# BUTSpeechFIT/DiariZen

Hardware: AMD Instinct MI355X
Metric: audio-seconds/s (RTF) for wavlm-large-s80 pipeline, 16 kHz mono (higher is better)
Workload: dtype f32 (operands split into 2 fp16 terms with exact power-of-two scaling = 22 significant bits, 3 fp16 MFMA products, fp32 accumulate: the error-corrected '3xFP16/3xTF32' scheme; kernels without an fp16 variant use the 3-term bf16 split)

## Files before the change

### diarizen_amd/_lib.py

```python
from __future__ import annotations

import ctypes as C
import os
from pathlib import Path

DZN_MAX_CONV = 8
DZN_MAX_LAYERS = 32
DZN_MAX_HEADS = 16

DZN_PREC_F32 = 0
DZN_PREC_BF16 = 1
DZN_PREC_F32_SPLIT = 2
DZN_PREC_F32_H2 = 3
DZN_PREC_F16 = 4

DZN_ACT_NONE, DZN_ACT_GELU, DZN_ACT_SWISH, DZN_ACT_RELU = 0, 1, 2, 3

DZN_F32, DZN_F64, DZN_I64 = 0, 1, 2

ERRORS = {0: "ok", -1: "invalid argument", -2: "out of memory", -3: "HIP runtime error",
          -4: "bad call order", -5: "missing state_dict key"}


class DznError(RuntimeError):
# ... 127 lines not shown
            f"{p} not found: build the HIP extension first (python -m diarizen_amd.build). "
            "diarizen_amd has no CPU fallback.")
    try:
        import torch
    except Exception:
        pass
    lib = C.CDLL(str(p))
    vp, i32, i64, f32 = C.c_void_p, C.c_int32, C.c_int64, C.c_float

    def sig(name, res, args):
        fn = getattr(lib, name)
        fn.restype = res
        fn.argtypes = args

    sig("dzn_create", i32, [C.POINTER(DznConfig), C.POINTER(vp)])
    sig("dzn_load_tensor", i32, [vp, C.c_char_p, vp, C.POINTER(i64), i32, i32])
    sig("dzn_finalize_weights", i32, [vp])
    sig("dzn_num_frames", i32, [vp, i32])
    sig("dzn_segment_forward", i32, [vp, vp, i32, i32, vp, vp, vp])
    sig("dzn_segment_forward_soft", i32, [vp, vp, i32, i32, vp, vp, vp, vp])
    sig("dzn_embed_forward", i32, [vp, vp, vp, i32, i32, i32, i32, vp, vp])
    sig("dzn_embed_forward_strided", i32, [vp, vp, i64, vp, i32, i32, i32, i32, vp, vp])
    sig("dzn_prepare_masks", i32, [vp, vp, i32, i32, i32, i32, i32, vp, vp, vp])
    sig("dzn_speaker_count", i32, [vp, i32, i32, i32, vp, i32, vp, vp, vp])
    sig("dzn_cluster_activations", i32, [vp, vp, i32, i32, i32, vp, i32, i32, vp, vp])
    sig("dzn_detect", i32, [vp, i32, i32, i32, vp, vp, i32, i32, f32, f32, vp, vp, vp])
    sig("dzn_detect_range", i32, [vp, i32, i32, i32, vp, vp, i32, i32, i32, f32, f32, vp, vp, vp, vp])
    sig("dzn_diarize_range", i32, [vp, vp, i32, i32, i32, vp, i32, i32, i32, i32, vp, vp, vp, vp])
    sig("dzn_diarize_range_scores", i32, [vp, vp, vp, i32, i32, i32, vp, vp, vp, i32, i32, i32, i32, vp, vp, vp, vp, vp])
    sig("dzn_speaker_scores", i32, [vp, vp, i32, i32, i32, vp, vp, vp, i32, i32, vp, vp])
    sig("dzn_match_counts", i32, [vp, vp, i32, i32, i32, i32, i32, vp, i32, i32, vp, vp])
    sig("dzn_debug_fetch", i32, [vp, C.c_char_p, vp, i64, C.POINTER(i64)])
    sig("dzn_embed_skip_stats", i32, [vp, C.POINTER(i64), C.POINTER(i64)])
    sig("dzn_num_ignored", i32, [vp])
    sig("dzn_workspace_bytes", i64, [vp])
    sig("dzn_last_error", C.c_char_p, [vp])
    sig("dzn_destroy", i32, [vp])
    sig("dzn_version", C.c_char_p, [])
    sig("dzn_profile_enable", i32, [i32])
    sig("dzn_profile_collect", i32, [C.POINTER(DznProfEntry), i32, C.POINTER(i32)])
    sig("dzn_profile_reserve", i32, [i32])
    sig("dzn_op_relpos_bucket", i32, [i32, i32, i32])
    sig("dzn_linkage_centroid", i32, [vp, i32, i32, vp, i32])
    sig("dzn_cdist_cosine", i32, [vp, i32, i32, vp, i32, vp, i32])
    sig("dzn_link_speakers", i32, [vp, vp, i32, i32, C.c_double, vp, C.POINTER(i32), i32])
    sig("dzn_link_speakers_last", i32, [C.POINTER(i64), C.POINTER(i32), C.POINTER(i32), C.POINTER(f32)])
# ... 74 lines not shown
    sig("dzn_op_ws_accum", i32, [vp, vp, f32, i32, i64, vp])
    sig("dzn_op_ws_sum", i32, [C.POINTER(vp), C.POINTER(f32), i32, vp, i64, vp])
    sig("dzn_op_col_scale", i32, [vp, i64, i32, i64, vp, vp])
    sig("dzn_op_layernorm_t", i32, [vp, i64, vp, i64, vp, vp, vp, i64, i32, i32, f32, i32, vp, i64, vp])
    sig("dzn_op_wave_stats", i32, [vp, i32, i32, f32, vp, vp])
    sig("dzn_op_frame_prep", i32, [vp, i32, i64, i32, i32, i32, i32, vp, f32, vp, vp])
    sig("dzn_op_power", i32, [vp, i64, i32, vp, vp])
    sig("dzn_op_log_cmn", i32, [vp, i32, i32, i32, f32, vp])
    sig("dzn_op_log_cmn_gather", i32, [vp, i32, vp, i32, i32, i32, f32, vp])
    sig("dzn_op_stem_conv", i32, [vp, i32, i32, i32, i32, vp, vp, vp, vp, vp, vp, vp])
    sig("dzn_op_stats_pool", i32, [vp, i32, i32, i32, i32, vp, i32, i32, vp, vp, vp])
    sig("dzn_op_window_active", i32, [vp, i32, i32, vp, vp])
    sig("dzn_op_compact_active", i32, [vp, i32, vp, vp, vp, vp])
    if hasattr(lib, "dzn_op_posconv_resident"):
        sig("dzn_op_pad_rows_split2", i32, [vp, vp, i64, i32, i32, i32, i32, i32, vp, vp, i32, i32, vp])
        sig("dzn_op_posconv_resident", i32, [C.POINTER(DznGemmDesc), i32, i32, i32, vp])
        sig("dzn_op_posconv_resident_fits", i32, [i32, i32, i32])
    _LIB = lib
    return lib


EXPORTED = [
    "dzn_create", "dzn_load_tensor", "dzn_finalize_weights", "dzn_num_frames",
    "dzn_segment_forward", "dzn_segment_forward_soft", "dzn_embed_forward", "dzn_embed_forward_strided", "dzn_prepare_masks", "dzn_speaker_count", "dzn_cluster_activations", "dzn_detect", "dzn_detect_range", "dzn_diarize_range", "dzn_diarize_range_scores", "dzn_speaker_scores", "dzn_match_counts", "dzn_debug_fetch", "dzn_embed_skip_stats", "dzn_num_ignored",
    "dzn_workspace_bytes", "dzn_last_error", "dzn_destroy", "dzn_version", "dzn_linkage_centroid", "dzn_cdist_cosine", "dzn_host_workspace_release",
    "dzn_host_workspace_bytes", "dzn_link_speakers", "dzn_link_speakers_last",
    "dzn_flac_info", "dzn_flac_decode", "dzn_resample", "dzn_resample_tile", "dzn_decode", "dzn_beamform_delays", "dzn_beamform_sum", "dzn_beamform_tile", "dzn_decode_planar", "dzn_beamform_track", "dzn_beamform_feed", "dzn_ingest_many", "dzn_beamform_many", "dzn_gather_windows", "dzn_vbx_create", "dzn_vbx_stats", "dzn_vbx_estep", "dzn_vbx_gamma", "dzn_vbx_destroy",
    "dzn_gallery_create", "dzn_gallery_put", "dzn_gallery_drop", "dzn_gallery_search", "dzn_gallery_geometry", "dzn_gallery_rows",
    "dzn_gallery_last_launch_ms", "dzn_gallery_destroy",
    "dzn_registry_create", "dzn_registry_append", "dzn_registry_match", "dzn_registry_rows", "dzn_registry_last_launch_ms",
    "dzn_registry_destroy",
    "dzn_op_gemm", "dzn_op_split_weights", "dzn_op_split_weights_h2", "dzn_op_split_weights_mx", "dzn_op_set_gemm_mx_cfg", "dzn_checked_status", "dzn_op_set_gemm_cfg", "dzn_op_amax", "dzn_op_conv3x3_c32", "dzn_op_conv3x3_c32_h2", "dzn_op_resblock32_fused", "dzn_op_resblock_ws", "dzn_op_set_resblock_np", "dzn_op_conv3x3_c32_ex", "dzn_op_resblock32_fused_ex", "dzn_op_resblock_ws_ex", "dzn_op_set_attention_noskip", "dzn_op_split_rows", "dzn_op_layernorm", "dzn_op_row_stats", "dzn_op_gate", "dzn_op_gate_stats", "dzn_op_gate_heads", "dzn_op_stats_finalize", "dzn_op_attention", "dzn_op_attention_h2", "dzn_op_attention_planes", "dzn_op_set_attention_qb", "dzn_op_set_attention_prefetch",
    "dzn_profile_enable", "dzn_profile_collect", "dzn_profile_reserve", "dzn_op_relpos_bucket",
    "dzn_op_glu_dwconv", "dzn_op_classify", "dzn_op_groupnorm_gelu", "dzn_op_gn_stats_floats", "dzn_op_pad_rows", "dzn_op_ws_accum",
    "dzn_op_ws_sum", "dzn_op_col_scale", "dzn_op_layernorm_t", "dzn_op_wave_stats", "dzn_op_frame_prep", "dzn_op_power",
    "dzn_op_log_cmn", "dzn_op_log_cmn_gather", "dzn_op_stem_conv", "dzn_op_stats_pool", "dzn_op_window_active",
    "dzn_op_compact_active", "dzn_op_pad_rows_split2", "dzn_op_posconv_resident", "dzn_op_posconv_resident_fits",
    "dzn_op_conv0_lnq", "dzn_op_conv0", "dzn_op_split_weights_h2_frag", "dzn_op_conv01_fused",
]


def profile_enable(on: bool) -> None:
    check(load().dzn_profile_enable(int(on)), None, "dzn_profile_enable")


def profile_reserve(n_events: int) -> None:
    check(load().dzn_profile_reserve(int(n_events)), None, "dzn_profile_reserve")
# ... 25 lines not shown
```

### diarizen_amd/csrc/common.h

```cpp
#pragma once
#include <hip/hip_runtime.h>
#include <stdint.h>
#include <math.h>
#include <string.h>
#include "../../include/dzn.h"
#include "../../include/dzn_ops.h"

typedef float f32x4 __attribute__((ext_vector_type(4)));
typedef __bf16 bf16x8 __attribute__((ext_vector_type(8)));
typedef __bf16 bf16x4 __attribute__((ext_vector_type(4)));
typedef unsigned short u16;

#define DZN_WAVE 64

template <int CTRL, int ROW_MASK>
__device__ __forceinline__ float dpp_add(float v) {
  const int t = __builtin_amdgcn_update_dpp(ROW_MASK == 0xF ? __float_as_int(v) : 0, __float_as_int(v), CTRL,
                                            ROW_MASK, 0xF, false);
  return v + __int_as_float(t);
}
__device__ __forceinline__ float wave_sum(float v) {
  v = dpp_add<0xB1, 0xF>(v);
  v = dpp_add<0x4E, 0xF>(v);
  v = dpp_add<0x124, 0xF>(v);
// ... 160 lines not shown

int launch_resblock32_fused(const float* in, float* out, const void* W1, const float* cs1, const float* b1, const void* W2,
                            const float* cs2, const float* b2, const float* amax_in, float* amax_out, float l1max1,
                            float bmax1, int B, int Hs, int Ws, int np, hipStream_t s, const int* z_count = nullptr,
                            const int* z_list = nullptr);

int launch_resblock_ws(const float* in, float* out, const void* W1, const float* cs1, const float* b1, const void* W2,
                       const float* cs2, const float* b2, const float* amax_in, float* amax_out, float l1max1, float bmax1,
                       int B, int Hs, int Ws, int C, hipStream_t s, const int* z_count = nullptr, const int* z_list = nullptr,
                       int np = 2);

int op_resblock_np();

int launch_prepare_masks(const uint8_t* ml, int B, int L, int S, int median, int exclude_overlap,
                         int min_num_frames, uint8_t* filtered, float* masks, hipStream_t st);

size_t resample_lds_bytes(int o, int n, int width);
int launch_resample(const void* src, int format, int channels, int channel, int64_t src_first, int64_t src_len, int64_t T,
                    const float* bank, int o, int n, int width, int64_t m0, int64_t m1, float* dst, hipStream_t st);
int launch_decode(const void* src, int format, int channels, int channel, int64_t frames, float* dst, hipStream_t st);
int launch_ingest_many(const void* stage, const dzn_ingest_desc* desc, int num_desc, int64_t tiles, size_t lds_bytes,
                       double bytes_moved, const float* banks, float* pool, hipStream_t st);
int launch_gather_windows(const float* pool, const int64_t* offsets, int B, int window, float* dst, hipStream_t st);
int launch_beamform_delays(const float* x, int channels, int64_t ch_stride, int64_t x_first, int64_t x_len, int64_t T, int ref,
                           int hop, int max_lag, const float* twiddle, int64_t b0, int64_t b1, int* lag, float* peak,
                           hipStream_t st);
int launch_beamform_sum(const float* x, int channels, int64_t ch_stride, int64_t x_first, int64_t x_len, int64_t T, int hop,
                        const int* delay, int64_t num_blocks, int64_t n0, int64_t n1, float* dst, hipStream_t st);
int launch_decode_planar(const void* src, int format, int channels, int64_t frames, float* dst, int64_t ch_stride,
                         hipStream_t st);
int launch_beamform_track(const int* lag, const float* peak, int64_t nblk, int channels, int ref, int hop, int64_t T,
                          float min_peak, int bound, int64_t b0, int64_t b1, int* state, int* delay, int64_t delay_stride,
                          hipStream_t st);
int launch_beamform_many(const void* stage, const dzn_beamform_desc* desc, int num_desc, int64_t decode_tiles, int64_t gcc_items,
                         int64_t sum_tiles, int max_hop, const double* work, const float* twiddles, float* planar,
                         int* lag, float* peak, int* state, int* delay, float* pool, float* beam, hipStream_t st);

bool prof_enabled();
int prof_begin(hipStream_t st, const char* cls, double flops, double bytes);
void prof_end(int id, hipStream_t st);

static inline bool first_use_on_device(unsigned long long& mask) {
  int dev = 0;
  (void)hipGetDevice(&dev);
  const unsigned long long bit = 1ull << (dev & 63);
  if (mask & bit) return false;
// ... 45 lines not shown
```

### diarizen_amd/csrc/engine.cpp

```cpp
#include <algorithm>
#include <cmath>
#include <cstdio>
#include <cstdlib>
#include <map>
#include <set>
#include <stdexcept>
#include <string>
#include <array>
#include <vector>

#include "common.h"

#define HIPCHK(x)                                                                        \
  do {                                                                                   \
    hipError_t e_ = (x);                                                                 \
    if (e_ != hipSuccess) {                                                              \
      throw EngineError(e_ == hipErrorOutOfMemory ? DZN_E_NOMEM : DZN_E_HIP,             \
                        std::string(#x) + ": " + hipGetErrorString(e_));                 \
    }                                                                                    \
  } while (0)

namespace {

struct EngineError : std::runtime_error {
// ... 73 lines not shown

std::string last_create_error;

enum F16Class { CLS_CONV, CLS_FEATPROJ, CLS_POSCONV, CLS_QKV, CLS_OUT, CLS_FFN1, CLS_FFN2, CLS_PROJ, CLS_CONF_W1, CLS_CONF_W2,
                CLS_CONF_QKV, CLS_CONF_OUT, CLS_CONF_PW1, CLS_CONF_PW2, CLS_RESNET };
const char* const F16_CLASSES[CLS_RESNET] = {"conv gemm", "feature projection", "pos conv", "qkv", "out_proj", "ffn1", "ffn2",
                                             "proj", "conf ffn w1", "conf ffn w2", "conf qkv", "conf out", "conf pw1", "conf pw2"};

struct Switches {
  bool fold_ln = true;
  bool conv0_quad_stats = true;
  bool fuse_conv01 = true;
  bool conv01_ln = true;
  bool ws_defer = true;
  bool att_planes = true;
  bool epilogue_stats = true;
  bool emb_skip = true;
  bool fuse_resblock = true;
  bool fuse_shortcut = true;
  bool posconv_resident = true;
  int resblock_ws = 2;
  unsigned f16_keep2 = 0x3f01;
  unsigned f16_mx = 0x3ffa;
  bool debug_taps = false;
};

Switches read_switches() {
  Switches s;
  s.fold_ln = !getenv("DZN_NO_LN_FOLD");
  s.conv0_quad_stats = !getenv("DZN_CONV0_WAVE_STATS");
  s.fuse_conv01 = !getenv("DZN_NO_CONV01_FUSION");
  s.conv01_ln = !getenv("DZN_CONV01_NO_LN");
  s.ws_defer = !getenv("DZN_NO_WS_DEFER");
  s.att_planes = !getenv("DZN_NO_ATT_PLANES");
  s.epilogue_stats = !getenv("DZN_NO_EPILOGUE_STATS");
  s.emb_skip = !getenv("DZN_EMB_NO_SKIP");
  s.fuse_resblock = !getenv("DZN_NO_RESBLOCK_FUSION");
  s.fuse_shortcut = !getenv("DZN_NO_SHORTCUT_FUSION");
  s.posconv_resident = !getenv("DZN_NO_POSCONV_RESIDENT");
  if (const char* e = getenv("DZN_RESBLOCK_WS")) s.resblock_ws = atoi(e);
  if (const char* e = getenv("DZN_F16_KEEP2")) s.f16_keep2 = (unsigned)strtoul(e, nullptr, 0);
  if (const char* e = getenv("DZN_F16_MX")) s.f16_mx = (unsigned)strtoul(e, nullptr, 0);
  const char* dbg = getenv("DZN_DEBUG_TAPS");
  s.debug_taps = dbg && dbg[0] == '1';
  return s;
}

}

struct dzn_handle {
  dzn_config cfg{};
  int device = 0;
  std::string err;
  std::map<std::string, HostT> sd;
  std::set<std::string> used;
  int ignored = 0;
  bool finalized = false;
  Switches sw;
  std::vector<void*> allocs;
  int64_t bytes = 0;
  std::map<std::string, std::vector<float>> taps;

// ... 47 lines not shown

  bool has_emb = false;
  float *hamming = nullptr;
  Lin dft, mel, seg1;
  float *stem_w = nullptr, *stem_b = nullptr;
  std::vector<std::vector<ResBlock>> stages;
  int emb_T = -1;
  int maxTf = 0;
  int sC[4]{};
  float* sbuf[4][3]{};
  int64_t sbuf_elems[4]{};
  struct EmbGeom {
    EmbStage stage[4]{};
  };
  std::map<int, EmbGeom> geoms;
  const EmbStage* stage = nullptr;
  float *frames = nullptr, *spec = nullptr, *pw = nullptr, *fb = nullptr, *pool = nullptr;
  int64_t fb_rows = 0;
  float* melg = nullptr;
  int *win_flag = nullptr, *win_idx = nullptr, *win_cnt = nullptr;
  long long* emb_totals = nullptr;
  long long emb_dense_windows = 0;
  bool mx_pack = false;
};

namespace {

using H = dzn_handle;

template <typename T>
T* dalloc(H* h, int64_t n, bool zero = true) {
  if (n <= 0) n = 1;
  void* p = nullptr;
  HIPCHK(hipMalloc(&p, n * sizeof(T)));
  h->allocs.push_back(p);
  h->bytes += n * (int64_t)sizeof(T);
  if (zero) HIPCHK(hipMemset(p, 0, n * sizeof(T)));
  return reinterpret_cast<T*>(p);
}

float* upload(H* h, const std::vector<float>& v) {
  float* p = dalloc<float>(h, (int64_t)v.size(), false);
  if (!v.empty()) HIPCHK(hipMemcpy(p, v.data(), v.size() * sizeof(float), hipMemcpyHostToDevice));
  return p;
}

// ... 407 lines not shown
    h->xpad3 = dalloc<u16>(h, 3 * h->xpad3_plane);
  }
  h->y = dalloc<float>(h, ML * D);
  h->ws = dalloc<float>(h, ML * D);
  h->xl_elems = (c.layer_norm_first && fold && c.n_layers > 0 && c.n_layers < WS_SUM_MAX && D % 4 == 0 &&
                 h->sw.ws_defer) ? (int64_t)c.n_layers * ML * D : 0;
  h->qkv = dalloc<float>(h, ML * 3 * maxQ);
  if (c.precision == DZN_PREC_F32_H2 && maxQ > 0 && h->sw.att_planes) {
    h->kvp_rows = ML + 64;
    h->kvp_ldmax = 2 * maxQ;
    h->kvp = dalloc<uint16_t>(h, 2 * h->kvp_rows * h->kvp_ldmax);
    h->kvs = dalloc<float>(h, h->kvp_rows * (h->kvp_ldmax / 64));
  }
  h->ao = dalloc<float>(h, ML * maxQ);
  h->gate = dalloc<float>(h, ML * h->H);
  h->mid = dalloc<float>(h, ML * maxF);
  h->hz = dalloc<float>(h, ML * A);
  h->ht = dalloc<float>(h, ML * A);
  h->hmid = dalloc<float>(h, ML * std::max(Fh, 3 * A));
  h->hv = dalloc<float>(h, ML * A);
  h->rstat = dalloc<float>(h, ML * 2);
  h->spart = dalloc<float>(h, ML * 32 * 2);
  h->amax = dalloc<float>(h, (int64_t)dzn_handle::AM_COUNT * c.max_batch);
}

void alloc_optional_workspace(H* h) {
  if (h->xl_elems <= 0) return;
  size_t free_b = 0, total_b = 0;
  if (hipMemGetInfo(&free_b, &total_b) != hipSuccess) return;
  const int64_t need = h->xl_elems * (int64_t)sizeof(float);
  const int64_t reserve = std::max<int64_t>((int64_t)32 << 30, (int64_t)(total_b / 4));
  if (need + reserve > (int64_t)free_b) return;
  void* p = nullptr;
  if (hipMalloc(&p, (size_t)need) != hipSuccess) {
    (void)hipGetLastError();
    return;
  }
  h->allocs.push_back(p);
  h->bytes += need;
  h->xl = reinterpret_cast<float*>(p);
}

constexpr int FB_FLEN = 400, FB_SHIFT = 160, FB_KP = 416, FB_NFFT = 512, FB_BINS = 256;

void stage_geometry(int NB, int T, const int* C, EmbStage* g) {
  for (int s = 0; s < 4; ++s) {
// ... 803 lines not shown

void emb_forward(H* h, const float* wave, int64_t win_stride, const float* masks, int B, int S, int N, int L, float* d_emb,
                 hipStream_t st) {
  if (N < FB_FLEN) throw EngineError(DZN_E_INVALID, "waveform shorter than one fbank frame (400 samples)");
  const int T = 1 + (N - FB_FLEN) / FB_SHIFT;
  if (T > h->maxTf) throw EngineError(DZN_E_INVALID, "N exceeds max_samples");
  if (S < 1 || S > 8) throw EngineError(DZN_E_INVALID, "S must be in [1, 8]");
  emb_set_geometry(h, T, st);
  const bool subset = h->sw.emb_skip && !h->sw.debug_taps && h->seg1.b != nullptr;
  const EmbCall e{h, st, B, T, S, L, subset ? h->win_cnt : nullptr, subset ? h->win_idx : nullptr, subset ? h->win_flag : nullptr};
  if (subset) {
    chk(launch_window_active(masks, B, S * L, h->win_flag, st), "window_active");
    chk(launch_compact_active(h->win_flag, B, h->win_cnt, h->win_idx, h->emb_totals, st), "compact_active");
  } else {
    h->emb_dense_windows += B;
  }
  emb_fbank(e, wave, win_stride, N);
  if (float* am0 = e.am(0, 0)) chk(launch_fill_u32(am0, 0u, 12 * (int64_t)h->cfg.max_batch, st), "image tracker reset");
  Img x = emb_stem(e);
  for (int s = 0; s < 4; ++s) x = emb_stage(e, s, x);
  emb_pool_head(e, x, masks, d_emb);
}

template <typename F>
int guarded(H* h, F&& f) {
  try {
    f();
    return DZN_OK;
  } catch (const EngineError& e) {
    if (h) h->err = e.what();
    else last_create_error = e.what();
    return e.code;
  } catch (const std::bad_alloc&) {
    if (h) h->err = "host allocation failed";
    return DZN_E_NOMEM;
  } catch (const std::exception& e) {
    if (h) h->err = e.what();
    return DZN_E_INVALID;
  }
}

}

void conv0_lnq_factor(const float* w, int C0, int k0, float* lq) {
  std::vector<double> wb(10, 0.0), Q(100, 0.0);
  for (int ch = 0; ch < C0; ++ch)
// ... 55 lines not shown
    last_create_error = "dzn_config.struct_size mismatch (ABI)";
    return DZN_E_INVALID;
  }
  if (cfg->precision == DZN_PREC_BF16) {
    last_create_error = "precision 1 (DZN_PREC_BF16) is not an engine mode: the bf16 engine was removed (reduced precision = DZN_PREC_F16)";
    return DZN_E_INVALID;
  }
  if (cfg->max_batch < 1 || cfg->max_samples < 400 ||
      (cfg->precision != DZN_PREC_F32 && cfg->precision != DZN_PREC_F32_SPLIT && cfg->precision != DZN_PREC_F32_H2 &&
       cfg->precision != DZN_PREC_F16)) {
    last_create_error = "bad max_batch / max_samples / precision";
    return DZN_E_INVALID;
  }
  int ndev = 0;
  if (hipGetDeviceCount(&ndev) != hipSuccess || ndev < 1) {
    last_create_error = "no HIP device visible (libdzn_hip has no CPU fallback)";
    return DZN_E_HIP;
  }
  dzn_handle* h = new (std::nothrow) dzn_handle();
  if (!h) return DZN_E_NOMEM;
  h->cfg = *cfg;
  if (hipGetDevice(&h->device) != hipSuccess) h->device = 0;
  h->sw = read_switches();
  *out = h;
  return DZN_OK;
}

int dzn_load_tensor(dzn_handle* h, const char* key, const void* host_ptr, const int64_t* shape,
                    int32_t ndim, int32_t dtype) {
  if (!h || !key || (!host_ptr && ndim > 0) || ndim < 0 || ndim > 8) return DZN_E_INVALID;
  if (h->finalized) {
    h->err = "dzn_load_tensor after dzn_finalize_weights";
    return DZN_E_STATE;
  }
  return guarded(h, [&] {
    HostT t;
    int64_t n = 1;
    for (int i = 0; i < ndim; ++i) {
      if (shape[i] < 0) throw EngineError(DZN_E_INVALID, "negative dimension");
      t.shape.push_back(shape[i]);
      n *= shape[i];
    }
    t.v.resize((size_t)n);
    if (dtype == DZN_F32) {
      memcpy(t.v.data(), host_ptr, (size_t)n * 4);
    } else if (dtype == DZN_F64) {
// ... 86 lines not shown
}

int dzn_prepare_masks(dzn_handle* h, const uint8_t* d_multilabel, int32_t B, int32_t L,
                      int32_t median_size, int32_t exclude_overlap, int32_t min_num_frames,
                      uint8_t* d_filtered, float* d_masks, void* hip_stream) {
  if (!h || !d_multilabel) return DZN_E_INVALID;
  if (!h->finalized) {
    h->err = "dzn_prepare_masks before dzn_finalize_weights";
    return DZN_E_STATE;
  }
  if (B < 1 || B > h->cfg.max_batch || L < 1 || (!d_filtered && !d_masks)) {
    h->err = "bad arguments to dzn_prepare_masks (B exceeds max_batch?)";
    return DZN_E_INVALID;
  }
  DeviceGuard dg(h->device);
  return guarded(h, [&] {
    chk(launch_prepare_masks(d_multilabel, B, L, h->cfg.max_speakers_per_chunk, median_size,
                             exclude_overlap, min_num_frames, d_filtered, d_masks,
                             reinterpret_cast<hipStream_t>(hip_stream)),
        "prepare_masks");
  });
}

int dzn_debug_fetch(dzn_handle* h, const char* name, float* host_out, int64_t cap, int64_t* n_elems) {
  if (!h || !name) return DZN_E_INVALID;
  auto it = h->taps.find(name);
  if (it == h->taps.end()) {
    h->err = std::string("no such tap (set DZN_DEBUG_TAPS=1 before dzn_create): ") + name;
    return DZN_E_INVALID;
  }
  if (n_elems) *n_elems = (int64_t)it->second.size();
  if (host_out) {
    if (cap < (int64_t)it->second.size()) return DZN_E_INVALID;
    memcpy(host_out, it->second.data(), it->second.size() * 4);
  }
  return DZN_OK;
}

int dzn_embed_skip_stats(const dzn_handle* h, int64_t* windows, int64_t* skipped) {
  if (!h) return DZN_E_INVALID;
  long long t[2] = {0, 0};
  if (h->emb_totals) {
    DeviceGuard dg(h->device);
    if (hipDeviceSynchronize() != hipSuccess ||
        hipMemcpy(t, h->emb_totals, sizeof(t), hipMemcpyDeviceToHost) != hipSuccess)
      return DZN_E_HIP;
  }
  t[0] += h->emb_dense_windows;
  if (windows) *windows = (int64_t)t[0];
  if (skipped) *skipped = (int64_t)t[1];
  return DZN_OK;
}

int dzn_num_ignored(const dzn_handle* h) { return h ? h->ignored : 0; }
int64_t dzn_workspace_bytes(const dzn_handle* h) { return h ? h->bytes : 0; }

const char* dzn_last_error(const dzn_handle* h) {
  return h ? h->err.c_str() : last_create_error.c_str();
}

int dzn_destroy(dzn_handle* h) {
  if (!h) return DZN_OK;
  DeviceGuard dg(h->device);
  for (void* p : h->allocs) (void)hipFree(p);
  delete h;
  return DZN_OK;
}

int dzn_resample(int32_t device, const void* d_src, int32_t src_format, int32_t channels, int32_t channel,
                 int64_t src_first_index, int64_t src_len, int64_t total_len, const float* d_bank, int32_t o, int32_t n,
                 int32_t width, int64_t m0, int64_t m1, float* d_dst, void* hip_stream) {
  auto refuse = [](const std::string& why) {
    last_create_error = "dzn_resample: " + why;
    return DZN_E_INVALID;
  };
  if (o < 1 || n < 1 || width < 0 || total_len < 0 || src_len < 0 || m0 < 0 || m1 < m0 || !d_bank)
    return refuse("bad o / n / width / lengths / range");
  if (src_format < 0 || src_format >= DZN_SRC_FORMATS || channels < 1)
    return refuse("src_format " + std::to_string(src_format) + " with " + std::to_string(channels) +
                  " channel(s): the formats are 0 (float32 mono) .. 7 (DZN_SRC_* of dzn.h), interleaved over channels >= 1");
  if (src_format == DZN_SRC_F32 && channels != 1)
    return refuse("src_format 0 is float32 mono, not " + std::to_string(channels) +
                  " channels (5 is float32 interleaved over channels)");
  if (channel < DZN_CHANNEL_DOWNMIX || channel >= channels)
    return refuse("channel " + std::to_string(channel) + " of a source with " + std::to_string(channels) + " channel(s)");
  if (total_len > INT64_MAX / n) return refuse("total_len * n overflows");
  if (src_len > INT64_MAX / 4 / channels) return refuse("src_len * channels * bytes per sample overflows");
// ... 558 lines not shown
```

### diarizen_amd/csrc/ingest.hip

```cpp
#include "common.h"
#include "checked.h"

DZN_CHECKED_TU(ingest)

#include "resample_tile.h"

namespace {

template <int FMT>
__device__ __forceinline__ void ingest_tile(const dzn_ingest_desc* __restrict__ d, const uint8_t* __restrict__ stage,
                                            const float* __restrict__ banks, float* __restrict__ pool, int tile, int lds_floats,
                                            float* __restrict__ xs) {
  const void* src = stage + d->src_offset;
  float* dst = pool + d->dst_offset;
  const int channels = d->channels, channel = d->channel;
  const int64_t m0 = d->m0, m1 = d->m1;
  if (d->bank_offset < 0) {
    const int64_t frames = m1 - m0;
    const int64_t r0 = (int64_t)tile * kResampleTile;
    const int64_t r1 = r0 + kResampleTile < frames ? r0 + kResampleTile : frames;
    DZN_CHECK(r0 < r1, 0x828, tile);
    for (int64_t r = r0 + threadIdx.x; r < r1; r += kThreads) decode_frame<FMT>(src, channels, channel, frames, r, dst);
    return;
  }
// ... 17 lines not shown
  while (lo < hi) {
    const int mid = (lo + hi + 1) >> 1;
    if (desc[mid].tile0 <= t) lo = mid; else hi = mid - 1;
  }
  const dzn_ingest_desc* d = desc + lo;
  const int tile = t - d->tile0;
  DZN_CHECK(tile >= 0 && (int64_t)tile * kResampleTile < d->m1 - d->m0, 0x829, lo);
  if (tile < 0 || (int64_t)tile * kResampleTile >= d->m1 - d->m0) return;
  switch (d->src_format) {
    case DZN_SRC_F32: ingest_tile<DZN_SRC_F32>(d, stage, banks, pool, tile, lds_floats, xs); break;
    case DZN_SRC_S16: ingest_tile<DZN_SRC_S16>(d, stage, banks, pool, tile, lds_floats, xs); break;
    case DZN_SRC_U8: ingest_tile<DZN_SRC_U8>(d, stage, banks, pool, tile, lds_floats, xs); break;
    case DZN_SRC_S24: ingest_tile<DZN_SRC_S24>(d, stage, banks, pool, tile, lds_floats, xs); break;
    case DZN_SRC_S32: ingest_tile<DZN_SRC_S32>(d, stage, banks, pool, tile, lds_floats, xs); break;
    case DZN_SRC_F32I: ingest_tile<DZN_SRC_F32I>(d, stage, banks, pool, tile, lds_floats, xs); break;
    case DZN_SRC_ULAW: ingest_tile<DZN_SRC_ULAW>(d, stage, banks, pool, tile, lds_floats, xs); break;
    case DZN_SRC_ALAW: ingest_tile<DZN_SRC_ALAW>(d, stage, banks, pool, tile, lds_floats, xs); break;
    default: DZN_CHECK(false, 0x82a, d->src_format); break;
  }
}

constexpr int kGatherVec = 4;

__global__ __launch_bounds__(kThreads) void gather_windows_kernel(const float* __restrict__ pool,
                                                                  const int64_t* __restrict__ offsets, int B, int window,
                                                                  float* __restrict__ dst, int bases_aligned) {
  const int b = (int)blockIdx.y;
  DZN_CHECK(b < B, 0x82b, b);
  const int64_t off = offsets[b], out = (int64_t)b * window;
  const float* __restrict__ s = pool + off;
  float* __restrict__ y = dst + out;
  const int stride = (int)gridDim.x * kThreads;
  const int first = (int)blockIdx.x * kThreads + (int)threadIdx.x;
  int done = 0;
  if (bases_aligned && !(off & (kGatherVec - 1)) && !(out & (kGatherVec - 1))) {
    const int nv = window / kGatherVec;
    const float4* __restrict__ s4 = reinterpret_cast<const float4*>(s);
    float4* __restrict__ y4 = reinterpret_cast<float4*>(y);
    for (int i = first; i < nv; i += stride) y4[i] = s4[i];
    done = nv * kGatherVec;
  }
  for (int i = done + first; i < window; i += stride) y[i] = s[i];
}

}

int launch_ingest_many(const void* stage, const dzn_ingest_desc* desc, int num_desc, int64_t tiles, size_t lds_bytes,
                       double bytes_moved, const float* banks, float* pool, hipStream_t st) {
  if (num_desc < 0 || tiles < 0 || tiles > 0x7fffffff || lds_bytes > kMaxLds) return DZN_E_INVALID;
  if (num_desc == 0 || tiles == 0) return DZN_OK;
  ProfScope prof_scope_(st, "ingest_many", 0.0, bytes_moved);
  hipLaunchKernelGGL(ingest_many_kernel, dim3((unsigned)tiles), dim3(kThreads), lds_bytes, st,
                     static_cast<const uint8_t*>(stage), desc, num_desc, banks, pool, (int)(lds_bytes / sizeof(float)));
  return hipGetLastError() == hipSuccess ? DZN_OK : DZN_E_HIP;
}

int launch_gather_windows(const float* pool, const int64_t* offsets, int B, int window, float* dst, hipStream_t st) {
  if (B < 0 || window < 1 || B > 65535) return DZN_E_INVALID;
  if (B == 0) return DZN_OK;
  ProfScope prof_scope_(st, "gather_windows", 0.0, 8.0 * (double)B * window);
  const int per_block = kThreads * kGatherVec;
  int gx = (window + per_block - 1) / per_block;
  gx = gx > 64 ? 64 : gx;
  const int aligned = !(reinterpret_cast<uintptr_t>(pool) & 15) && !(reinterpret_cast<uintptr_t>(dst) & 15);
  hipLaunchKernelGGL(gather_windows_kernel, dim3((unsigned)gx, (unsigned)B), dim3(kThreads), 0, st, pool, offsets, B, window,
                     dst, aligned);
  return hipGetLastError() == hipSuccess ? DZN_OK : DZN_E_HIP;
}
```

### diarizen_amd/engine.py

```python
from __future__ import annotations

import ctypes as C
from typing import Dict, Mapping, Optional

import numpy as np
import torch

from . import _lib
from ._lib import (DZN_F32, DZN_F64, DZN_I64, DZN_PREC_F32, DZN_PREC_F32_SPLIT, DznConfig,
                   check)
from .configs import EmbConfig, SegConfig

PRECISIONS = {"f32": DZN_PREC_F32, "fp32": DZN_PREC_F32,
              "f32s": DZN_PREC_F32_SPLIT, "f32_split": DZN_PREC_F32_SPLIT, "f32h": _lib.DZN_PREC_F32_H2,
              "f16": _lib.DZN_PREC_F16, "fp16": _lib.DZN_PREC_F16}


def make_dzn_config(seg: SegConfig, emb: Optional[EmbConfig], max_batch: int, max_samples: int,
                    precision: str = "f32h") -> DznConfig:
    c = DznConfig()
    c.struct_size = C.sizeof(DznConfig)
    c.precision = PRECISIONS[precision]
    c.max_batch = int(max_batch)
    c.max_samples = int(max_samples)
# ... 135 lines not shown
        _, S, L = masks.shape
        out = torch.empty((B, S, self.emb.embed_dim), device=views.device, dtype=torch.float32)
        check(self.lib.dzn_embed_forward_strided(self._h, C.c_void_p(views.data_ptr()), stride,
                                                 C.c_void_p(masks.data_ptr()), B, S, N, L,
                                                 C.c_void_p(out.data_ptr()), self._stream()),
              self._h, "dzn_embed_forward_strided")
        return out

    def prepare_masks(self, multilabel: torch.Tensor, median_size: int = 11,
                      exclude_overlap: bool = True, min_num_frames: int = -1,
                      want_masks: bool = True):
        assert multilabel.is_cuda and multilabel.dtype == torch.uint8 and multilabel.is_contiguous()
        B, L, S = multilabel.shape
        filt = torch.empty_like(multilabel)
        masks = (torch.empty((B, S, L), device=multilabel.device, dtype=torch.float32)
                 if want_masks else None)
        check(self.lib.dzn_prepare_masks(self._h, C.c_void_p(multilabel.data_ptr()), B, L,
                                         int(median_size), int(exclude_overlap), int(min_num_frames),
                                         C.c_void_p(filt.data_ptr()),
                                         C.c_void_p(masks.data_ptr()) if masks is not None else None,
                                         self._stream()), self._h, "dzn_prepare_masks")
        return filt, masks

    def debug_fetch(self, name: str) -> np.ndarray:
        n = C.c_int64(0)
        check(self.lib.dzn_debug_fetch(self._h, name.encode(), None, 0, C.byref(n)), self._h,
              f"dzn_debug_fetch({name})")
        out = np.empty(n.value, dtype=np.float32)
        check(self.lib.dzn_debug_fetch(self._h, name.encode(), C.c_void_p(out.ctypes.data), n.value,
                                       C.byref(n)), self._h, f"dzn_debug_fetch({name})")
        return out

    def embed_skip_stats(self):
        w, k = C.c_int64(0), C.c_int64(0)
        check(self.lib.dzn_embed_skip_stats(self._h, C.byref(w), C.byref(k)), self._h, "dzn_embed_skip_stats")
        return w.value, k.value

    def close(self) -> None:
        if getattr(self, "_h", None) is not None and self._h.value:
            self.lib.dzn_destroy(self._h)
            self._h = C.c_void_p()

    def __del__(self):
        try:
            self.close()
        except Exception:
# ... 2 lines not shown
```

### diarizen_amd/inference.py

```python
from __future__ import annotations

import math
from dataclasses import dataclass
from typing import Optional, Tuple

import torch

from contextlib import nullcontext as _nullcontext

from .engine import Engine


def window_plan(num_samples: int, window: int, step: int) -> Tuple[int, bool]:
    if num_samples >= window:
        num_chunks = (num_samples - window) // step + 1
        has_last = (num_samples - window) % step > 0
    else:
        num_chunks = 0
        has_last = True
    return num_chunks, has_last


FBANK_FRAME, FBANK_SHIFT = 400, 160

# ... 104 lines not shown
        views = self.windows_view(wave)
        c0, c1 = window_range if window_range is not None else (0, views.shape[0])
        n_full, has_last = window_plan(wave.numel(), self.window, self.step)
        return self.run_views(views, c0, c1, with_embeddings=with_embeddings, hook=hook, with_scores=with_scores,
                              dense_from=n_full if has_last else None)

    def run_views(self, views: torch.Tensor, c0: int, c1: int, with_embeddings: bool = True, hook=None,
                  with_scores: bool = False, dense_from: Optional[int] = None) -> SlideResult:
        eng = self.engine
        wave = views
        C = max(c1 - c0, 0)
        S = eng.seg.max_speakers_per_chunk
        seg = torch.empty((C, self.num_frames, S), device=wave.device, dtype=torch.uint8)
        emb = (torch.empty((C, S, eng.emb.embed_dim), device=wave.device, dtype=torch.float32)
               if with_embeddings else None)
        soft = torch.empty((C, self.num_frames, S), device=wave.device, dtype=torch.float32) if with_scores else None
        nb = max(1, -(-C // self.batch_size))
        bs = max(1, -(-C // nb))
        if hook is not None:
            hook(completed=0, total=C)
        if nb > 1 and hook is None and len(self.engines) < self._max_engines:
            self._grow(wave.device)
        multi = len(self.engines) > 1 and hook is None and nb > 1
        cur = torch.cuda.current_stream(wave.device)
        if multi:
            if self._streams is None:
                self._streams = [torch.cuda.Stream(device=wave.device) for _ in self.engines]
            for st in self._streams:
                st.wait_stream(cur)
        for bi, s0 in enumerate(range(c0, c1, bs)):
            s1 = min(s0 + bs, c1)
            k = bi % len(self.engines) if multi else 0
            e = self.engines[k]
            with torch.cuda.stream(self._streams[k]) if multi else _nullcontext():
                chunk = views[s0:s1].contiguous()
                if with_scores:
                    _, ml, soft[s0 - c0:s1 - c0] = e.segment(chunk, want_logp=False, want_soft=True)
                else:
                    _, ml = e.segment(chunk, want_logp=False)
                filt, masks = e.prepare_masks(ml, self.median_size, self.exclude_overlap,
                                              self.min_num_frames if self.exclude_overlap else -1,
                                              want_masks=with_embeddings)
                seg[s0 - c0:s1 - c0] = filt
                if with_embeddings:
                    ns, nd = embed_routes(s0, s1, c1 if dense_from is None else dense_from)
                    if ns:
# ... 11 lines not shown
```

### include/dzn.h

```cpp
#ifndef DZN_H_
#define DZN_H_

#include <stdint.h>
#include <stddef.h>

#ifdef __cplusplus
extern "C" {
#endif

#define DZN_MAX_CONV 8
#define DZN_MAX_LAYERS 32
#define DZN_MAX_HEADS 16

#define DZN_OK 0
#define DZN_E_INVALID (-1)
#define DZN_E_NOMEM (-2)
#define DZN_E_HIP (-3)
#define DZN_E_STATE (-4)
#define DZN_E_MISSING (-5)

#define DZN_F32 0
#define DZN_F64 1
#define DZN_I64 2

// ... 53 lines not shown
                    const int64_t* shape, int32_t ndim, int32_t dtype);

int dzn_finalize_weights(dzn_handle* h);

int dzn_num_frames(const dzn_handle* h, int32_t num_samples);

int dzn_segment_forward(dzn_handle* h, const float* d_wave, int32_t B, int32_t N,
                        float* d_logp, uint8_t* d_multilabel, void* hip_stream);

int dzn_segment_forward_soft(dzn_handle* h, const float* d_wave, int32_t B, int32_t N,
                             float* d_logp, uint8_t* d_multilabel, float* d_soft, void* hip_stream);

int dzn_embed_forward(dzn_handle* h, const float* d_wave, const float* d_masks,
                      int32_t B, int32_t S, int32_t N, int32_t L, float* d_emb,
                      void* hip_stream);

int dzn_embed_forward_strided(dzn_handle* h, const float* d_rec, int64_t win_stride, const float* d_masks,
                              int32_t B, int32_t S, int32_t N, int32_t L, float* d_emb,
                              void* hip_stream);

int dzn_prepare_masks(dzn_handle* h, const uint8_t* d_multilabel, int32_t B, int32_t L,
                      int32_t median_size, int32_t exclude_overlap, int32_t min_num_frames,
                      uint8_t* d_filtered, float* d_masks, void* hip_stream);

int dzn_speaker_count(const uint8_t* d_seg, int32_t C, int32_t L, int32_t S, const int32_t* d_start_frame, int32_t T,
                      int32_t* d_work, uint8_t* d_count, void* hip_stream);
int dzn_cluster_activations(const uint8_t* d_seg, const int8_t* d_hard, int32_t C, int32_t L, int32_t S,
                            const int32_t* d_start_frame, int32_t T, int32_t K, int32_t* d_act, void* hip_stream);

int dzn_detect(const uint8_t* d_seg, int32_t C, int32_t L, int32_t S, const int32_t* d_start_frame, const double* d_weight,
               int32_t T, int32_t tasks, float onset, float offset, float* d_scores, uint8_t* d_active, void* hip_stream);

int dzn_detect_range(const uint8_t* d_seg, int32_t C, int32_t L, int32_t S, const int32_t* d_start_frame,
                     const double* d_weight, int32_t t0, int32_t t1, int32_t tasks, float onset, float offset,
                     const uint8_t* d_entry, float* d_scores, uint8_t* d_active, void* hip_stream);

int dzn_diarize_range(const uint8_t* d_seg, const int8_t* d_hard, int32_t C, int32_t L, int32_t S,
                      const int32_t* d_start_frame, int32_t t0, int32_t t1, int32_t K, int32_t max_count,
                      uint8_t* d_count, uint8_t* d_active, int32_t* d_act, void* hip_stream);

int dzn_diarize_range_scores(const uint8_t* d_seg, const int8_t* d_hard, const float* d_soft, int32_t C, int32_t L, int32_t S,
                             const int32_t* d_start_frame, const double* d_hamming, const double* d_warm_up, int32_t t0,
                             int32_t t1, int32_t K, int32_t max_count, uint8_t* d_count, uint8_t* d_active, int32_t* d_act,
                             float* d_scores, void* hip_stream);

int dzn_speaker_scores(const float* d_soft, const int8_t* d_hard, int32_t C, int32_t L, int32_t S,
// ... 168 lines not shown
```

Measured before the change: 1859.

## Move sliding-window loop into C with side-stream overlap of embedding and segmentation

Adds dzn_slide_forward, which runs the per-batch segmentation, mask preparation and embedding loop inside the library. It copies strided window views with a new kernel and runs the embedding model on a side stream, double-buffering masks so the next batch's segmentation overlaps the current batch's embeddings. The Python single-engine path now calls it instead of looping per batch, which also removes per-batch Python and launch overhead. In exchange it adds events, a second stream and extra workspace, and ordering is more complex because of the dense-buffer reuse waits.

```diff
diff --git a/diarizen_amd/_lib.py b/diarizen_amd/_lib.py
--- a/diarizen_amd/_lib.py
+++ b/diarizen_amd/_lib.py
@@ -173,6 +173,7 @@
     sig("dzn_embed_forward", i32, [vp, vp, vp, i32, i32, i32, i32, vp, vp])
     sig("dzn_embed_forward_strided", i32, [vp, vp, i64, vp, i32, i32, i32, i32, vp, vp])
     sig("dzn_prepare_masks", i32, [vp, vp, i32, i32, i32, i32, i32, vp, vp, vp])
+    sig("dzn_slide_forward", i32, [vp, vp, i64, i32, i32, i32, i32, i32, i32, i32, vp, vp, vp, vp])
     sig("dzn_speaker_count", i32, [vp, i32, i32, i32, vp, i32, vp, vp, vp])
     sig("dzn_cluster_activations", i32, [vp, vp, i32, i32, i32, vp, i32, i32, vp, vp])
     sig("dzn_detect", i32, [vp, i32, i32, i32, vp, vp, i32, i32, f32, f32, vp, vp, vp])
@@ -293,7 +294,7 @@
 
 EXPORTED = [
     "dzn_create", "dzn_load_tensor", "dzn_finalize_weights", "dzn_num_frames",
-    "dzn_segment_forward", "dzn_segment_forward_soft", "dzn_embed_forward", "dzn_embed_forward_strided", "dzn_prepare_masks", "dzn_speaker_count", "dzn_cluster_activations", "dzn_detect", "dzn_detect_range", "dzn_diarize_range", "dzn_diarize_range_scores", "dzn_speaker_scores", "dzn_match_counts", "dzn_debug_fetch", "dzn_embed_skip_stats", "dzn_num_ignored",
+    "dzn_segment_forward", "dzn_segment_forward_soft", "dzn_embed_forward", "dzn_embed_forward_strided", "dzn_prepare_masks", "dzn_slide_forward", "dzn_speaker_count", "dzn_cluster_activations", "dzn_detect", "dzn_detect_range", "dzn_diarize_range", "dzn_diarize_range_scores", "dzn_speaker_scores", "dzn_match_counts", "dzn_debug_fetch", "dzn_embed_skip_stats", "dzn_num_ignored",
     "dzn_workspace_bytes", "dzn_last_error", "dzn_destroy", "dzn_version", "dzn_linkage_centroid", "dzn_cdist_cosine", "dzn_host_workspace_release",
     "dzn_host_workspace_bytes", "dzn_link_speakers", "dzn_link_speakers_last",
     "dzn_flac_info", "dzn_flac_decode", "dzn_resample", "dzn_resample_tile", "dzn_decode", "dzn_beamform_delays", "dzn_beamform_sum", "dzn_beamform_tile", "dzn_decode_planar", "dzn_beamform_track", "dzn_beamform_feed", "dzn_ingest_many", "dzn_beamform_many", "dzn_gather_windows", "dzn_vbx_create", "dzn_vbx_stats", "dzn_vbx_estep", "dzn_vbx_gamma", "dzn_vbx_destroy",
diff --git a/diarizen_amd/csrc/common.h b/diarizen_amd/csrc/common.h
--- a/diarizen_amd/csrc/common.h
+++ b/diarizen_amd/csrc/common.h
@@ -206,6 +206,7 @@
 int launch_ingest_many(const void* stage, const dzn_ingest_desc* desc, int num_desc, int64_t tiles, size_t lds_bytes,
                        double bytes_moved, const float* banks, float* pool, hipStream_t st);
 int launch_gather_windows(const float* pool, const int64_t* offsets, int B, int window, float* dst, hipStream_t st);
+int launch_strided_windows(const float* src, int64_t row_stride, int B, int window, float* dst, hipStream_t st);
 int launch_beamform_delays(const float* x, int channels, int64_t ch_stride, int64_t x_first, int64_t x_len, int64_t T, int ref,
                            int hop, int max_lag, const float* twiddle, int64_t b0, int64_t b1, int* lag, float* peak,
                            hipStream_t st);
diff --git a/diarizen_amd/csrc/engine.cpp b/diarizen_amd/csrc/engine.cpp
--- a/diarizen_amd/csrc/engine.cpp
+++ b/diarizen_amd/csrc/engine.cpp
@@ -119,6 +119,7 @@
   int resblock_ws = 2;
   unsigned f16_keep2 = 0x3f01;
   unsigned f16_mx = 0x3ffa;
+  bool slide_overlap = true;
   bool debug_taps = false;
 };
 
@@ -135,6 +136,7 @@
   s.fuse_resblock = !getenv("DZN_NO_RESBLOCK_FUSION");
   s.fuse_shortcut = !getenv("DZN_NO_SHORTCUT_FUSION");
   s.posconv_resident = !getenv("DZN_NO_POSCONV_RESIDENT");
+  s.slide_overlap = !getenv("DZN_NO_SLIDE_OVERLAP");
   if (const char* e = getenv("DZN_RESBLOCK_WS")) s.resblock_ws = atoi(e);
   if (const char* e = getenv("DZN_F16_KEEP2")) s.f16_keep2 = (unsigned)strtoul(e, nullptr, 0);
   if (const char* e = getenv("DZN_F16_MX")) s.f16_mx = (unsigned)strtoul(e, nullptr, 0);
@@ -228,6 +230,12 @@
   long long* emb_totals = nullptr;
   long long emb_dense_windows = 0;
   bool mx_pack = false;
+
+  hipStream_t side = nullptr;
+  hipEvent_t ev_in = nullptr, ev_masks[2]{}, ev_emb[2]{};
+  uint8_t* slide_ml = nullptr;
+  float* slide_masks[2]{};
+  float* slide_dense = nullptr;
 };
 
 namespace {
@@ -681,6 +689,8 @@
   h->rstat = dalloc<float>(h, ML * 2);
   h->spart = dalloc<float>(h, ML * 32 * 2);
   h->amax = dalloc<float>(h, (int64_t)dzn_handle::AM_COUNT * c.max_batch);
+  h->slide_ml = dalloc<uint8_t>(h, ML * c.max_speakers_per_chunk);
+  for (float*& m : h->slide_masks) m = dalloc<float>(h, ML * c.max_speakers_per_chunk);
 }
 
 void alloc_optional_workspace(H* h) {
@@ -1530,6 +1540,68 @@
   emb_pool_head(e, x, masks, d_emb);
 }
 
+struct SlideArgs {
+  const float* wave;
+  int64_t win_stride;
+  int N, C, dense_from, batch;
+  int median, exclude_overlap, min_num_frames;
+  uint8_t* seg;
+  float* emb;
+  float* soft;
+};
+
+void slide_forward(H* h, const SlideArgs& a, int L, hipStream_t st) {
+  const dzn_config& c = h->cfg;
+  const int S = c.max_speakers_per_chunk;
+  const int nb = (a.C + a.batch - 1) / a.batch, bs = (a.C + nb - 1) / nb;
+  hipStreamCaptureStatus cap = hipStreamCaptureStatusNone;
+  HIPCHK(hipStreamIsCapturing(st, &cap));
+  const bool overlap = a.emb && nb > 1 && h->sw.slide_overlap && !h->sw.debug_taps && cap == hipStreamCaptureStatusNone;
+  if (!h->slide_dense) h->slide_dense = dalloc<float>(h, (int64_t)c.max_batch * c.max_samples, false);
+  float* dense = h->slide_dense;
+  int side_last = -1;
+  bool dense_busy = false;
+  if (overlap) {
+    HIPCHK(hipEventRecord(h->ev_in, st));
+    HIPCHK(hipStreamWaitEvent(h->side, h->ev_in, 0));
+  }
+  try {
+    for (int i = 0, s0 = 0; s0 < a.C; ++i, s0 += bs) {
+      const int n = std::min(bs, a.C - s0), k = i & 1;
+      const float* rows = a.wave + (int64_t)s0 * a.win_stride;
+      const int64_t o = (int64_t)s0 * L * S;
+      if (dense_busy) HIPCHK(hipStreamWaitEvent(st, h->ev_emb[k ^ 1], 0));
+      chk(launch_strided_windows(rows, a.win_stride, n, a.N, dense, st), "strided_windows");
+      seg_forward(h, dense, n, a.N, nullptr, h->slide_ml, a.soft ? a.soft + o : nullptr, st);
+      if (overlap && i >= 2) HIPCHK(hipStreamWaitEvent(st, h->ev_emb[k], 0));
+      float* masks = a.emb ? h->slide_masks[k] : nullptr;
+      chk(launch_prepare_masks(h->slide_ml, n, L, S, a.median, a.exclude_overlap, a.min_num_frames, a.seg + o, masks, st),
+          "prepare_masks");
+      if (!a.emb) continue;
+      hipStream_t lane = overlap ? h->side : st;
+      if (overlap) {
+        HIPCHK(hipEventRecord(h->ev_masks[k], st));
+        HIPCHK(hipStreamWaitEvent(lane, h->ev_masks[k], 0));
+      }
+      const int ns = std::min(std::max(a.dense_from - s0, 0), n), nd = n - ns;
+      float* e = a.emb + (int64_t)s0 * S * c.embed_out_dim;
+      if (ns) emb_forward(h, rows, ns > 1 ? a.win_stride : a.N, masks, ns, S, a.N, L, e, lane);
+      if (nd)
+        emb_forward(h, dense + (int64_t)ns * a.N, a.N, masks + (int64_t)ns * S * L, nd, S, a.N, L,
+                    e + (int64_t)ns * S * c.embed_out_dim, lane);
+      if (overlap) {
+        HIPCHK(hipEventRecord(h->ev_emb[k], lane));
+        side_last = k;
+        dense_busy = nd > 0;
+      }
+    }
+  } catch (...) {
+    if (overlap && hipEventRecord(h->ev_emb[0], h->side) == hipSuccess) (void)hipStreamWaitEvent(st, h->ev_emb[0], 0);
+    throw;
+  }
+  if (side_last >= 0) HIPCHK(hipStreamWaitEvent(st, h->ev_emb[side_last], 0));
+}
+
 template <typename F>
 int guarded(H* h, F&& f) {
   try {
@@ -1631,6 +1703,14 @@
   h->cfg = *cfg;
   if (hipGetDevice(&h->device) != hipSuccess) h->device = 0;
   h->sw = read_switches();
+  bool ok = hipStreamCreateWithFlags(&h->side, hipStreamNonBlocking) == hipSuccess;
+  for (hipEvent_t* e : {&h->ev_in, &h->ev_masks[0], &h->ev_masks[1], &h->ev_emb[0], &h->ev_emb[1]})
+    ok = ok && hipEventCreateWithFlags(e, hipEventDisableTiming) == hipSuccess;
+  if (!ok) {
+    last_create_error = "could not create the side stream / events of dzn_slide_forward";
+    dzn_destroy(h);
+    return DZN_E_HIP;
+  }
   *out = h;
   return DZN_OK;
 }
@@ -1763,6 +1843,37 @@
   });
 }
 
+int dzn_slide_forward(dzn_handle* h, const float* d_wave, int64_t win_stride, int32_t N, int32_t C, int32_t dense_from,
+                      int32_t batch, int32_t median_size, int32_t exclude_overlap, int32_t min_num_frames, uint8_t* d_seg,
+                      float* d_emb, float* d_soft, void* hip_stream) {
+  if (!h) return DZN_E_INVALID;
+  if (!h->finalized || (d_emb && !h->has_emb)) {
+    h->err = "dzn_slide_forward before dzn_finalize_weights / embeddings asked of a handle without the embedding model";
+    return DZN_E_STATE;
+  }
+  const int L = dzn_num_frames(h, N), S = h->cfg.max_speakers_per_chunk;
+  const char* why = nullptr;
+  if (C < 0) why = "C < 0";
+  else if (batch < 1 || batch > h->cfg.max_batch) why = "batch outside [1, max_batch]";
+  else if (N < 1 || N > h->cfg.max_samples || L < 1) why = "N outside the handle's window lengths";
+  else if (win_stride < 0) why = "negative win_stride";
+  else if (dense_from < 0) why = "negative dense_from";
+  else if (C > 0 && (!d_wave || !d_seg)) why = "null d_wave / d_seg";
+  else if (S < 1 || S > 8 || (median_size > 1 && !(median_size & 1)) || 2 * (((size_t)L * S + 3) & ~(size_t)3) + 32 > 64 * 1024)
+    why = "median_size / S / L the masks stage refuses";
+  else if (d_emb && (N < FB_FLEN || 1 + (N - FB_FLEN) / FB_SHIFT > h->maxTf)) why = "N outside what the embedding model takes";
+  if (why) {
+    h->err = std::string("bad arguments to dzn_slide_forward: ") + why;
+    return DZN_E_INVALID;
+  }
+  if (C == 0) return DZN_OK;
+  DeviceGuard dg(h->device);
+  return guarded(h, [&] {
+    const SlideArgs a{d_wave, win_stride, N, C, dense_from, batch, median_size, exclude_overlap, min_num_frames, d_seg, d_emb, d_soft};
+    slide_forward(h, a, L, reinterpret_cast<hipStream_t>(hip_stream));
+  });
+}
+
 int dzn_debug_fetch(dzn_handle* h, const char* name, float* host_out, int64_t cap, int64_t* n_elems) {
   if (!h || !name) return DZN_E_INVALID;
   auto it = h->taps.find(name);
@@ -1803,7 +1914,13 @@
 int dzn_destroy(dzn_handle* h) {
   if (!h) return DZN_OK;
   DeviceGuard dg(h->device);
+  if (h->side) {
+    (void)hipStreamSynchronize(h->side);
+    (void)hipStreamDestroy(h->side);
+  }
   for (void* p : h->allocs) (void)hipFree(p);
+  for (hipEvent_t e : {h->ev_in, h->ev_masks[0], h->ev_masks[1], h->ev_emb[0], h->ev_emb[1]})
+    if (e) (void)hipEventDestroy(e);
   delete h;
   return DZN_OK;
 }
diff --git a/diarizen_amd/csrc/ingest.hip b/diarizen_amd/csrc/ingest.hip
--- a/diarizen_amd/csrc/ingest.hip
+++ b/diarizen_amd/csrc/ingest.hip
@@ -63,18 +63,11 @@
 
 constexpr int kGatherVec = 4;
 
-__global__ __launch_bounds__(kThreads) void gather_windows_kernel(const float* __restrict__ pool,
-                                                                  const int64_t* __restrict__ offsets, int B, int window,
-                                                                  float* __restrict__ dst, int bases_aligned) {
-  const int b = (int)blockIdx.y;
-  DZN_CHECK(b < B, 0x82b, b);
-  const int64_t off = offsets[b], out = (int64_t)b * window;
-  const float* __restrict__ s = pool + off;
-  float* __restrict__ y = dst + out;
+__device__ __forceinline__ void copy_window_row(const float* __restrict__ s, float* __restrict__ y, int window, bool vec) {
   const int stride = (int)gridDim.x * kThreads;
   const int first = (int)blockIdx.x * kThreads + (int)threadIdx.x;
   int done = 0;
-  if (bases_aligned && !(off & (kGatherVec - 1)) && !(out & (kGatherVec - 1))) {
+  if (vec) {
     const int nv = window / kGatherVec;
     const float4* __restrict__ s4 = reinterpret_cast<const float4*>(s);
     float4* __restrict__ y4 = reinterpret_cast<float4*>(y);
@@ -82,6 +75,23 @@
     done = nv * kGatherVec;
   }
   for (int i = done + first; i < window; i += stride) y[i] = s[i];
+}
+
+__global__ __launch_bounds__(kThreads) void gather_windows_kernel(const float* __restrict__ pool,
+                                                                  const int64_t* __restrict__ offsets, int B, int window,
+                                                                  float* __restrict__ dst, int bases_aligned) {
+  const int b = (int)blockIdx.y;
+  DZN_CHECK(b < B, 0x82b, b);
+  const int64_t off = offsets[b], out = (int64_t)b * window;
+  copy_window_row(pool + off, dst + out, window, bases_aligned && !(off & (kGatherVec - 1)) && !(out & (kGatherVec - 1)));
+}
+
+__global__ __launch_bounds__(kThreads) void strided_windows_kernel(const float* __restrict__ src, int64_t row_stride, int B,
+                                                                   int window, float* __restrict__ dst, int bases_aligned) {
+  const int b = (int)blockIdx.y;
+  DZN_CHECK(b < B, 0x82c, b);
+  const int64_t off = (int64_t)b * row_stride, out = (int64_t)b * window;
+  copy_window_row(src + off, dst + out, window, bases_aligned && !(off & (kGatherVec - 1)) && !(out & (kGatherVec - 1)));
 }
 
 }
@@ -108,3 +118,16 @@
                      dst, aligned);
   return hipGetLastError() == hipSuccess ? DZN_OK : DZN_E_HIP;
 }
+
+int launch_strided_windows(const float* src, int64_t row_stride, int B, int window, float* dst, hipStream_t st) {
+  if (B < 0 || window < 1 || B > 65535 || row_stride < 0) return DZN_E_INVALID;
+  if (B == 0) return DZN_OK;
+  ProfScope prof_scope_(st, "strided_windows", 0.0, 8.0 * (double)B * window);
+  const int per_block = kThreads * kGatherVec;
+  int gx = (window + per_block - 1) / per_block;
+  gx = gx > 64 ? 64 : gx;
+  const int aligned = !(reinterpret_cast<uintptr_t>(src) & 15) && !(reinterpret_cast<uintptr_t>(dst) & 15);
+  hipLaunchKernelGGL(strided_windows_kernel, dim3((unsigned)gx, (unsigned)B), dim3(kThreads), 0, st, src, row_stride, B, window,
+                     dst, aligned);
+  return hipGetLastError() == hipSuccess ? DZN_OK : DZN_E_HIP;
+}
diff --git a/diarizen_amd/engine.py b/diarizen_amd/engine.py
--- a/diarizen_amd/engine.py
+++ b/diarizen_amd/engine.py
@@ -181,6 +181,23 @@
                                          self._stream()), self._h, "dzn_prepare_masks")
         return filt, masks
 
+    def slide(self, views: torch.Tensor, seg: torch.Tensor, emb: Optional[torch.Tensor] = None,
+              soft: Optional[torch.Tensor] = None, *, batch: int, dense_from: Optional[int] = None, median_size: int = 11,
+              exclude_overlap: bool = True, min_num_frames: int = -1) -> None:
+        assert views.is_cuda and views.dtype == torch.float32 and views.dim() == 2 and views.stride(1) == 1
+        C_, N = views.shape
+        L, S = self.num_frames(N), self.seg.max_speakers_per_chunk
+        stride = int(views.stride(0)) if C_ > 1 else N
+        assert seg.is_cuda and seg.dtype == torch.uint8 and seg.shape == (C_, L, S) and seg.is_contiguous()
+        assert emb is None or (emb.is_cuda and emb.dtype == torch.float32 and emb.shape == (C_, S, self.emb.embed_dim)
+                               and emb.is_contiguous())
+        assert soft is None or (soft.is_cuda and soft.dtype == torch.float32 and soft.shape == seg.shape and soft.is_contiguous())
+        check(self.lib.dzn_slide_forward(
+            self._h, C.c_void_p(views.data_ptr()), stride, N, C_, C_ if dense_from is None else int(dense_from), int(batch),
+            int(median_size), int(exclude_overlap), int(min_num_frames), C.c_void_p(seg.data_ptr()),
+            C.c_void_p(emb.data_ptr()) if emb is not None else None,
+            C.c_void_p(soft.data_ptr()) if soft is not None else None, self._stream()), self._h, "dzn_slide_forward")
+
     def debug_fetch(self, name: str) -> np.ndarray:
         n = C.c_int64(0)
         check(self.lib.dzn_debug_fetch(self._h, name.encode(), None, 0, C.byref(n)), self._h,
diff --git a/diarizen_amd/inference.py b/diarizen_amd/inference.py
--- a/diarizen_amd/inference.py
+++ b/diarizen_amd/inference.py
@@ -150,6 +150,12 @@
         if nb > 1 and hook is None and len(self.engines) < self._max_engines:
             self._grow(wave.device)
         multi = len(self.engines) > 1 and hook is None and nb > 1
+        if hook is None and not multi:
+            eng.slide(views[c0:c1], seg, emb, soft, batch=self.batch_size, median_size=self.median_size,
+                      dense_from=None if dense_from is None else min(max(dense_from - c0, 0), C),
+                      exclude_overlap=self.exclude_overlap,
+                      min_num_frames=self.min_num_frames if self.exclude_overlap else -1)
+            return SlideResult(seg, emb, self.window, self.step, self.num_frames, soft)
         cur = torch.cuda.current_stream(wave.device)
         if multi:
             if self._streams is None:
diff --git a/include/dzn.h b/include/dzn.h
--- a/include/dzn.h
+++ b/include/dzn.h
@@ -99,6 +99,10 @@
 int dzn_prepare_masks(dzn_handle* h, const uint8_t* d_multilabel, int32_t B, int32_t L,
                       int32_t median_size, int32_t exclude_overlap, int32_t min_num_frames,
                       uint8_t* d_filtered, float* d_masks, void* hip_stream);
+
+int dzn_slide_forward(dzn_handle* h, const float* d_wave, int64_t win_stride, int32_t N, int32_t C, int32_t dense_from,
+                      int32_t batch, int32_t median_size, int32_t exclude_overlap, int32_t min_num_frames, uint8_t* d_seg,
+                      float* d_emb, float* d_soft, void* hip_stream);
 
 int dzn_speaker_count(const uint8_t* d_seg, int32_t C, int32_t L, int32_t S, const int32_t* d_start_frame, int32_t T,
                       int32_t* d_work, uint8_t* d_count, void* hip_stream);
```

Result: no change. 1869 (median of 6 runs) (+0.5%).
